# jp-schneider/awesome

Hardware: AMD Instinct MI355X
Metric: INR-fits/sec (256x256 grid, convexity prior) (higher is better)
Workload: dtype f32; 1 GPU; 1 x 256x256 synthetic convex blob per GPU, ConvexNextNet(h=130,L=1), SE(sigmoid) mean, Adam lr 2e-3, clamp, E=2000 full-batch steps (BASELINE configs[1]); images_per_gpu=1, grid=256x256, epochs_per_fit=2000, parallelism=dp1 (independent fits)

## Files before the change

awesome_amd/csrc/flow.h:

```cpp
#pragma once
#include "icnn_step.h"
#include <stdlib.h>

namespace {

constexpr float LEAKY_SLOPE = 0.01f;

struct FlowMap {
    int W, K;
    int nb_stride;
    int p_nb, p_scale, FP;
    int e_cp_stride;
    int e_nb, e_scale, FE;
    float slope;
};

__host__ __device__ inline FlowMap make_flow_map(int W, int K, float slope = LEAKY_SLOPE) {
    FlowMap m;
    m.W = W;
    m.K = K;
    m.slope = slope;
    m.nb_stride = 3 * W + 3;
    m.p_nb = 6;
    m.p_scale = m.p_nb + 2 * K * m.nb_stride;
// ... 514 lines not shown
    float* opt;
    float* grads_out;
    const float* slab1;
    const float* slab2;
    const float* lr_hdr;
    long long hdr_stride;
    InrOptDesc opt_desc;
    FlowMap m;
    int blocks1, S1, chunks, Wp;
    int t;
    double bc1;
    float bc2_sqrt, one_minus_b1, one_minus_b2, wd_g;
    int mode;
    const int32_t* status;
    const float* gscale;
    const float* loss_slabs;
    int loss_wgs;
    long long loss_PS;
};

__device__ __forceinline__ float block_sum256(float v, float* sm, const int tid) {
    v = sum_over_groups(sum_over_points(v));
    __syncthreads();
    if ((tid & 63) == 0) sm[tid >> 6] = v;
    __syncthreads();
    return ((sm[0] + sm[1]) + sm[2]) + sm[3];
}
__device__ __forceinline__ float block_sum256(float v, float* sm) { return block_sum256(v, sm, threadIdx.x); }

constexpr int LOSS_GROUPS = 16;
__device__ __forceinline__ float loss_column_group_sum(const float* __restrict__ sl, const int wgs, const size_t PS, const int grp) {
    float lp = 0.f;
    int w = grp;
    for (; w + 15 * LOSS_GROUPS < wgs; w += 16 * LOSS_GROUPS) {
        float q[16];
#pragma unroll
        for (int k = 0; k < 16; ++k) q[k] = sl[(size_t)(w + k * LOSS_GROUPS) * PS];
#pragma unroll
        for (int k = 0; k < 16; ++k) lp += q[k];
    }
    for (; w < wgs; w += LOSS_GROUPS) lp += sl[(size_t)w * PS];
    return lp;
}

__device__ __forceinline__ bool frozen_in_launch(const float* __restrict__ loss_slabs, const int wgs, const long long PS,
                                                 const float* __restrict__ hdr0, const long long hdr_stride, const int t, const int img,
                                                 const int tid) {
    __shared__ float redl[LOSS_GROUPS];
    if (tid < LOSS_GROUPS) redl[tid] = loss_column_group_sum(loss_slabs + (size_t)img * wgs * PS, wgs, (size_t)PS, tid);
    __syncthreads();
    float loss_now = 0.f;
#pragma unroll
    for (int k = 0; k < LOSS_GROUPS; ++k) loss_now += redl[k];
    const bool bad_before = hdr0 != nullptr && hdr0[(size_t)img * hdr_stride + 6 + (t & 1)] != 0.f;
    return bad_before || !isfinite(loss_now);
}

__device__ __forceinline__ float adam_apply(const FlowUpdArgs& u, float gmul, float p, float g, float lr, float wd, float* m_, float* v_) {
    g = g * gmul;
    if (wd != 0.f) g = __fadd_rn(g, __fmul_rn(wd, p));
    float m = *m_, v = *v_;
    m = __fadd_rn(m, __fmul_rn(u.one_minus_b1, __fsub_rn(g, m)));
    v = __fadd_rn(__fmul_rn(v, u.opt_desc.beta2), __fmul_rn(__fmul_rn(u.one_minus_b2, g), g));
    const float step_size = (float)((double)lr / u.bc1);
    const float denom = __fadd_rn(__fdiv_rn(__fsqrt_rn(v), u.bc2_sqrt), u.opt_desc.eps);
    *m_ = m;
    *v_ = v;
    return __fadd_rn(p, __fdiv_rn(__fmul_rn(-step_size, m), denom));
}

template <int BATCH>
__device__ __forceinline__ void flow_update_body(const FlowUpdArgs& u, const int nb, const int img, const int tid) {
    __shared__ float sm[4];
    const float gmul = u.gscale != nullptr ? u.gscale[img] : 1.f;
    const FlowMap& m = u.m;
    const bool frozen = !isfinite(gmul) ||
                        ((u.mode == 0 && u.loss_slabs != nullptr)
                             ? frozen_in_launch(u.loss_slabs, u.loss_wgs, u.loss_PS, u.lr_hdr, u.hdr_stride, u.t, img, tid)
                             : ((u.lr_hdr != nullptr && u.lr_hdr[(size_t)img * u.hdr_stride + 6 + ((u.t + 1) & 1)] != 0.f) ||
                                (u.status != nullptr && u.status[img] != INR_STATUS_OK)));
    const int mode = (u.mode == 0 && frozen) ? 2 : u.mode;
    const int W = m.W, K = m.K;
    float* __restrict__ fp = u.FP + (size_t)img * m.FP;
    float* __restrict__ fe = u.FE + (size_t)img * m.FE;
    float* __restrict__ om = u.opt ? u.opt + (size_t)img * 2 * m.FP : nullptr;
    float* __restrict__ ov = om ? om + m.FP : nullptr;
    float* __restrict__ go = u.grads_out ? u.grads_out + (size_t)img * m.FP : nullptr;
    const float lr = u.lr_hdr ? u.lr_hdr[(size_t)img * u.hdr_stride + (u.t & 1)] : u.opt_desc.lr;
    if (nb < 2 * K) {
        const int pb = m.p_nb + nb * m.nb_stride;
        const int eb = m.e_nb + (nb >> 1) * m.e_cp_stride + (nb & 1);
        const int i = nb >> 1, net = nb & 1;
        const bool on = tid < W;
// ... 144 lines not shown
```

awesome_amd/csrc/icnn_step.h:

```cpp
#pragma once
#include <hip/hip_runtime.h>
#include <stdint.h>
#include <math.h>

#include <type_traits>

#include "inrfit.h"

typedef float f32x4 __attribute__((ext_vector_type(4)));
typedef float f32x2 __attribute__((ext_vector_type(2)));

#define MFMA16(a, b, c) __builtin_amdgcn_mfma_f32_16x16x4f32((a), (b), (c), 0, 0, 0)
__device__ __forceinline__ float relu0(float x) { return __int_as_float(max(__float_as_int(x), 0)); }
constexpr float INV_2PI = 0.15915494309189535f;
__device__ __forceinline__ float hw_sin(float x) { return __builtin_amdgcn_sinf(__builtin_amdgcn_fractf(x * INV_2PI)); }
__device__ __forceinline__ float hw_cos(float x) { return __builtin_amdgcn_cosf(__builtin_amdgcn_fractf(x * INV_2PI)); }
template <int ACT>
__device__ __forceinline__ float act0_f(float pre, float omega) {
    if constexpr (ACT == INR_ACT_COS) return hw_cos(pre);
    else if constexpr (ACT == INR_ACT_SIN) return hw_sin(omega * pre);
    else return relu0(pre);
}
template <int ACT>
__device__ __forceinline__ float dact0_f(float pre, float omega) {
// ... 164 lines not shown
        }
    }
    if (j < m.p_bo) {
        slot[0] = m.off_wo + (j - m.p_wo);
        return 1;
    }
    slot[0] = m.off_sc + (j - m.p_bo);
    return 1;
}

struct StepArgs {
    const float* wimg;
    const float* targets;
    const float* coef;
    float* slabs;
    float* logits;
    float* dcoords;
    InrGridDesc grid;
    long long N;
    int n_images, wgs, PS, loss_kind;
    float act_omega;
    const float* seg;
    float c_align;
    int data_count;
    int use_noneclass;
    float noneclass;
    int align_soft;
    int align_begin;
};

// ... 722 lines not shown
        }
        for (int i = tid; i < HM * NEXT; i += WG_THREADS) {
            const int row = i / NEXT, e = i - row * NEXT;
            const float v = wsum(SC_L0 + row * 4 + e);
            if (e == 0) slab[G::SL_TILE + G::P_BIN + row] = v;
            else slab[G::SL_TILE + G::P_WIN + row * C + (e - 1)] = v;
        }
        if (tid < HR * NEXT) {
            const int u = tid / NEXT, e = tid - u * NEXT;
            const float v = wsum(SC_L0L + u * 4 + e);
            if (e == 0) slab[G::SL_TILE + G::P_BIN + HM + u] = v;
            else slab[G::SL_TILE + G::P_WIN + (HM + u) * C + (e - 1)] = v;
        }
        if (tid < 2 + C) {
            const float v = wsum(SC_SC + tid);
            if (tid == 0) slab[G::SL_LOSS] = v;
            else if (tid == 1) slab[G::slab_col(G::P_BO)] = v;
            else slab[G::slab_col(G::P_SO) + tid - 2] = v;
        }
    }
#if INR_STAMPS
    if (TRAIN && (tid & 63) == 0 && blockIdx.x < 1024) {
        __builtin_amdgcn_s_waitcnt(0);
        const unsigned long long rt_end = __builtin_amdgcn_s_memrealtime();
        if (tid == 0) {
            g_wgtimes[blockIdx.x][0] = rt_entry;
            g_wgtimes[blockIdx.x][1] = rt_loop;
            g_wgtimes[blockIdx.x][2] = rt_loop_end;
        }
        atomicMax(&g_wgtimes[blockIdx.x][3], rt_end);
    }
    if (TRAIN && blockIdx.x == 0 && tid == 0) {
// ... 13 lines not shown
```

awesome_amd/csrc/icnn_step2.h:

```cpp
#pragma once
#include "icnn_step.h"


namespace {

template <int H, int C>
struct Cfg2 {
    using G1 = Cfg<H, C>;
    static constexpr int TM = G1::TM, HM = G1::HM, HR = G1::HR, NEXT = G1::NEXT, NRL = G1::NRL, KG = G1::KG, PT = G1::PT;
    static constexpr int S = G1::S, SA = G1::SA, SB = G1::SB, RPW = G1::RPW;
    static constexpr int ext_pos(int e) { return G1::ext_pos(e); }
    static constexpr int nr_in(int tk) { return G1::nr_in(tk); }
    static constexpr int OFF_SC = 0;
    static constexpr int OFF_WINE = OFF_SC + 8;
    static constexpr int OFF_WIN = OFF_WINE + 4 * PT;
    static constexpr int OFF_BIN = OFF_WIN + C * 16;
    static constexpr int OFF_FLOOR = OFF_BIN + 16;
    static constexpr int OFF_WO = OFF_FLOOR + 16;
    static constexpr int OFF_WCT0 = OFF_WO + PT;
    static constexpr int OFF_WCT1 = OFF_WCT0 + HR * PT;
    static constexpr int WREG = round_up(H * S + 16, 256);
    static constexpr int OFF_W0 = round_up(OFF_WCT1 + HR * PT, 4);
    static constexpr int OFF_W1 = OFF_W0 + WREG;
    static constexpr int IMG_FLOATS = OFF_W1 + WREG;
// ... 705 lines not shown
        }
        for (int i = tid; i < HM * NEXT; i += WG_THREADS) {
            const int row = i / NEXT, e = i - row * NEXT;
            const float v = wsum(SC_L0 + row * 4 + e);
            if (e == 0) slab[G::SL_IN + G::P_BIN + row] = v;
            else slab[G::SL_IN + G::P_WIN + row * C + (e - 1)] = v;
        }
        if (tid < HR * NEXT) {
            const int u = tid / NEXT, e = tid - u * NEXT;
            const float v = wsum(SC_L0L + u * 4 + e);
            if (e == 0) slab[G::SL_IN + G::P_BIN + HM + u] = v;
            else slab[G::SL_IN + G::P_WIN + (HM + u) * C + (e - 1)] = v;
        }
        if (tid < 2 + C) {
            const float v = wsum(SC_SC + tid);
            if (tid == 0) slab[G::SL_LOSS] = v;
            else if (tid == 1) slab[G::SL_WO + (G::P_BO - G::P_WO)] = v;
            else slab[G::SL_WO + (G::P_SO - G::P_WO) + tid - 2] = v;
        }
    }
}

}
```

awesome_amd/csrc/inrfit.hip:

```cpp
#include "icnn_step.h"
#include "icnn_step2.h"
#include "flow.h"
#include "rnvp.h"
#include "joint_loss.h"
#include "wide.h"
#include "star.h"
#include "cnnseg.h"
#include "fcseg.h"

#include <type_traits>
#include <vector>

namespace {

constexpr int UPD_RANGES = WIDE_MAX_LAYERS + 1;
struct UpdArgs {
    float* wimg;
    ImgMap img;
    float* params;
    float* opt_state;
    const float* slabs;
    float* loss_hist;
    float* grads_out;
    float* loss_out;
    int32_t* status;
    InrOptDesc opt;
    int P, PS, wgs, n_images;
    int Pu, hu;
    int t;
    double bc1;
    float bc2_sqrt;
    float one_minus_b1, one_minus_b2;
    int hist_idx, hist_stride;
    int mode;
    int clamp_lo[UPD_RANGES], clamp_hi[UPD_RANGES];
    int freeze_lo[UPD_RANGES], freeze_hi[UPD_RANGES];
// ... 26 lines not shown
        if (j < m.p_s[k] + H * C) {
            const int q = j - m.p_s[k], o = q / C;
            return o < h ? base_u + h * h + h + q : -1;
        }
    }
    if (j < m.p_bo) {
        const int i = j - m.p_wo;
        return i < h ? base_u + i : -1;
    }
    return base_u + h + (j - m.p_bo);
}

constexpr int UPD_MAX_PARAMS = 256;
constexpr int UPD_GROUPS = 16;

inline int upd_params_per_block(int cols, int reserve = 0) {
    const int cus = 256 - reserve;
    int ppb = ((cols + cus - 1) / cus + 3) / 4 * 4;
    if (ppb < 16) ppb = 16;
    if (ppb > UPD_MAX_PARAMS) ppb = UPD_MAX_PARAMS;
    return ppb;
}
inline dim3 upd_grid(int cols, int n_images, int reserve = 0) {
    const int ppb = upd_params_per_block(cols, reserve);
    return dim3((cols + ppb - 1) / ppb, n_images);
}
inline dim3 upd_block(int cols, int reserve = 0) { return dim3(upd_params_per_block(cols, reserve) / 4, UPD_GROUPS); }

#if INR_STAMPS
__device__ unsigned long long g_updtimes[512][4];
#define UPD_STAMP(k)                                                                                          \
    if (threadIdx.x == 0 && threadIdx.y == 0 && img == 0 && bx < 512) {                                       \
        __builtin_amdgcn_s_waitcnt(0);                                                                        \
        g_updtimes[bx][k] = __builtin_amdgcn_s_memrealtime();                                                 \
    }
#else
#define UPD_STAMP(k)
#endif
static_assert(UPD_GROUPS == LOSS_GROUPS, "the loss column is summed in the update's group order");
__device__ __forceinline__ void icnn_update_body(const UpdArgs& u, const int bx, const int img) {
    const int tx = threadIdx.x, grp = threadIdx.y;
    const int ppb = 4 * blockDim.x;
    __shared__ float red[UPD_GROUPS][UPD_MAX_PARAMS];
    __shared__ float redl[UPD_GROUPS];
    UPD_STAMP(0);
    const int jl = grp * blockDim.x + tx;
    const int j = jl < ppb ? slab_param_of_col(u.img, bx * ppb + jl) : -1;
    const int ju = (j >= 0 && j < u.P) ? user_param_index(u.img, u.hu, j) : -1;
    float* __restrict__ st = u.opt_state + (size_t)img * (2 * (size_t)u.Pu + INR_OPT_HEADER_FLOATS);
    float* __restrict__ hdr = st + 2 * (size_t)u.Pu;
    float p_old = 0.f, m_old = 0.f, v_old = 0.f, lr_now = 0.f;
    bool bad_before = false;
    if (u.mode == 0 && j >= 0) {
        bad_before = hdr[6 + (u.t & 1)] != 0.f;
        lr_now = hdr[u.t & 1];
        if (ju >= 0) {
            p_old = u.params[(size_t)img * u.Pu + ju];
            m_old = st[ju];
            v_old = st[u.Pu + ju];
        }
    }
    {
        const int j4 = bx * ppb + 4 * tx;
        f32x4 part = f32x4{0.f, 0.f, 0.f, 0.f};
        if (j4 < u.PS && slab_param_of_col(u.img, j4) >= 0) {
            const float* __restrict__ sl = u.slabs + (size_t)img * u.wgs * u.PS + j4;
            int w = grp;
            for (; w + 15 * UPD_GROUPS < u.wgs; w += 16 * UPD_GROUPS) {
                f32x4 q[16];
#pragma unroll
                for (int k = 0; k < 16; ++k) q[k] = *(const f32x4*)(sl + (size_t)(w + k * UPD_GROUPS) * u.PS);
#pragma unroll
                for (int k = 0; k < 16; ++k) part += q[k];
            }
            for (; w < u.wgs; w += UPD_GROUPS) part += *(const f32x4*)(sl + (size_t)w * u.PS);
        }
        *(f32x4*)&red[grp][4 * tx] = part;
        if (u.mode == 0 && tx == 0) {
            redl[grp] = loss_column_group_sum(u.slabs + (size_t)img * u.wgs * u.PS + (u.img.sl_cols - 1), u.wgs, (size_t)u.PS, grp);
        }
    }
    UPD_STAMP(1);
    __syncthreads();
    if (j < 0) return;
    float gsum = 0.f;
#pragma unroll
    for (int k = 0; k < UPD_GROUPS; ++k) gsum += red[k][jl];
    if (u.gscale != nullptr && j < u.P) gsum *= u.gscale[img];

    UPD_STAMP(2);
    if (u.mode == 1) {
        if (ju >= 0) u.grads_out[(size_t)img * u.Pu + ju] = gsum;
        else if (j == u.P) u.loss_out[img] = gsum;
        return;
// ... 64 lines not shown
        if (in) p = fmaxf(p, 0.f);
    }
    u.params[(size_t)img * u.Pu + ju] = p;
    if (u.wimg != nullptr) {
        int slot[2];
        const int ns = image_slots(u.img, j, slot);
        float* __restrict__ wi = u.wimg + (size_t)img * u.img.floats;
        wi[slot[0]] = p;
        if (ns > 1) wi[slot[1]] = p;
    }
    st[ju] = m;
    st[u.Pu + ju] = v;
    UPD_STAMP(3);
}

__global__ __launch_bounds__(UPD_MAX_PARAMS / 4 * UPD_GROUPS) void icnn_update_kernel(const UpdArgs u) { icnn_update_body(u, blockIdx.x, blockIdx.y); }

constexpr int UPD_UNION_MAX_THREADS = 768;
__global__ __launch_bounds__(UPD_UNION_MAX_THREADS) void cdn_update_kernel(const UpdArgs ui, const FlowUpdArgs uf, const int nbi) {
    if ((int)blockIdx.x < nbi) {
        icnn_update_body(ui, blockIdx.x, blockIdx.y);
        return;
    }
    const int tid = threadIdx.y * blockDim.x + threadIdx.x;
    if (tid >= 256) return;
    flow_update_body<32>(uf, (int)blockIdx.x - nbi, blockIdx.y, tid);
}
template <int C>
__global__ __launch_bounds__(UPD_UNION_MAX_THREADS) void pcn_update_kernel(const UpdArgs ui, const RnvpUpdArgs ur, const int nbi) {
    if ((int)blockIdx.x < nbi) {
        icnn_update_body(ui, blockIdx.x, blockIdx.y);
        return;
    }
    const int tid = threadIdx.y * blockDim.x + threadIdx.x;
    if (tid >= 256) return;
    rnvp_update_body<C>(ur, (int)blockIdx.x - nbi, blockIdx.y, tid);
}
inline bool upd_union_ok(int cols, int reserve) {
    const dim3 b = upd_block(cols, reserve);
    const int n = (int)(b.x * b.y);
    static const bool off = getenv("INRFIT_SPLIT_UPDATES") != nullptr;
    return !off && n >= 256 && n <= UPD_UNION_MAX_THREADS;
}

__global__ __launch_bounds__(256) void pack_image_kernel(float* __restrict__ wimg, const ImgMap m) {
    float* __restrict__ dst = wimg + (size_t)blockIdx.y * m.floats;
// ... 238 lines not shown
        return INR_ELAUNCH;
    for (int k = 1; k < 3; ++k) {
        if (hipFuncSetAttribute((const void*)e->train_act[k], hipFuncAttributeMaxDynamicSharedMemorySize, e->lds_bytes) != hipSuccess ||
            hipFuncSetAttribute((const void*)e->fwd_act[k], hipFuncAttributeMaxDynamicSharedMemorySize, e->lds_bytes) != hipSuccess)
            return INR_ELAUNCH;
    }
    return INR_OK;
}

constexpr int INR_SLAB_BUFFERS = 4;

struct Workspace {
    float* coef;
    float* wimg;
    float* slabs;
    float* slabs0;
    long long slab_floats;
    int wgs, PS;
    long long bytes;
    void set_step(int it) { slabs = slabs0 + (size_t)(it % INR_SLAB_BUFFERS) * slab_floats; }
    int act0 = INR_ACT_RELU;
    float act_omega = 0.f;
    int hu = 0, Pu = 0;
    void set_user(const KernelEntry* e, const InrModelDesc* m) {
        hu = m ? m->n_hidden : e->h;
        const long long h = hu, c = e->c, l = e->l;
        Pu = (int)(h * c + h + l * (h * h + h + h * c) + h + 1 + c);
    }
};

Workspace carve(const KernelEntry* e, long long n_points, int n_images, void* base) {
    Workspace w;
    w.wgs = wgs_per_image(n_points, n_images);
    w.PS = (e->img.sl_cols + 31) / 32 * 32;
    const long long coef_bytes = ((long long)n_images * 2 * 4 + 255) / 256 * 256;
    const long long img_bytes = ((long long)n_images * e->img.floats * 4 + 255) / 256 * 256;
    w.slab_floats = ((long long)n_images * w.wgs * w.PS + 63) / 64 * 64;
    const long long slab_bytes = w.slab_floats * 4 * INR_SLAB_BUFFERS;
    w.coef = (float*)base;
    w.wimg = (float*)((char*)base + coef_bytes);
    w.slabs0 = w.slabs = (float*)((char*)base + coef_bytes + img_bytes);
    w.bytes = coef_bytes + img_bytes + slab_bytes;
    return w;
}

}

__global__ __launch_bounds__(256) void mfma_stream_kernel(float* __restrict__ sink, int iters) {
    f32x4 acc[8];
#pragma unroll
    for (int t = 0; t < 8; ++t) acc[t] = f32x4{0.f, 0.f, 0.f, 0.f};
    f32x4 av[8], bv;
    unsigned h = (blockIdx.x * 256u + threadIdx.x) * 2654435761u + 12345u;
    auto rnd = [&]() { h = h * 1664525u + 1013904223u; return (float)(int)(h >> 8) * (1.f / 8388608.f) - 1.f; };
#pragma unroll
    for (int t = 0; t < 8; ++t)
// ... 323 lines not shown
                       int loss_kind, int n_images, float* logits, hipStream_t s, float* dcoords = nullptr,
                       const float* align_seg = nullptr, float c_align = 0.f, const StepMask& mask = StepMask{}) {
    StepArgs a{};
    a.dcoords = dcoords;
    a.seg = align_seg;
    a.c_align = c_align;
    a.data_count = (int)(mask.data_count > 0 ? mask.data_count : grid->n_points);
    a.use_noneclass = mask.use_noneclass;
    a.noneclass = mask.noneclass;
    a.align_soft = mask.align_soft;
    a.align_begin = (int)mask.align_begin;
    a.wimg = w.wimg;
    a.targets = targets;
    a.coef = w.coef;
    a.slabs = w.slabs;
    a.logits = logits;
    a.grid = *grid;
    a.N = grid->n_points;
    a.n_images = n_images;
    a.wgs = w.wgs;
    a.PS = w.PS;
    a.loss_kind = loss_kind;
    a.act_omega = w.act_omega;
    if (dcoords && w.act0 != INR_ACT_RELU) return INR_EUNSUPPORTED;
    hipLaunchKernelGGL(train ? (dcoords ? e->train_dx : e->train_act[w.act0]) : e->fwd_act[w.act0], dim3((unsigned)(n_images * w.wgs)),
                       dim3(WG_THREADS), e->lds_bytes, s, a);
    return hipGetLastError() == hipSuccess ? INR_OK : INR_ELAUNCH;
}

struct StepTiming {
// ... 21 lines not shown
static int check_loss(const InrLossDesc* l) {
    if (!l) return INR_EINVAL;
    if (l->kind != INR_LOSS_SE && l->kind != INR_LOSS_BCE && l->kind != INR_LOSS_EXTERNAL) return INR_EINVAL;
    if (l->weight_mode < INR_WEIGHT_NONE || l->weight_mode > INR_WEIGHT_EXPLICIT) return INR_EINVAL;
    return INR_OK;
}

static UpdArgs make_upd_args(const KernelEntry* e, const Workspace& w, float* params, float* opt_state, float* loss_hist,
                             int32_t* status, const InrOptDesc* opt, int n_images, int steps) {
    UpdArgs u{};
    u.wimg = w.wimg;
    u.img = e->img;
    u.params = params;
    u.opt_state = opt_state;
    u.slabs = w.slabs;
    u.loss_hist = loss_hist;
    u.status = status;
    u.opt = *opt;
    u.P = e->P;
    u.Pu = w.Pu;
    u.hu = w.hu;
    u.PS = w.PS;
    u.wgs = w.wgs;
    u.n_images = n_images;
    u.hist_stride = steps;
    u.one_minus_b1 = (float)(1.0 - (double)opt->beta1);
    u.one_minus_b2 = (float)(1.0 - (double)opt->beta2);
    u.mode = 0;
    for (int k = 0; k < UPD_RANGES; ++k) u.clamp_lo[k] = u.clamp_hi[k] = 0;
    for (int k = 0; k < e->img.L; ++k) {
// ... 13 lines not shown
    return u;
}

static void bias_corrections(const InrOptDesc* opt, int t, double* bc1, float* bc2_sqrt) {
    *bc1 = 1.0 - pow((double)opt->beta1, (double)t);
    *bc2_sqrt = (float)sqrt(1.0 - pow((double)opt->beta2, (double)t));
}

static void set_step_consts(UpdArgs& u, const InrOptDesc* opt, int t, int hist_idx = 0) {
    u.t = t;
    bias_corrections(opt, t, &u.bc1, &u.bc2_sqrt);
    u.hist_idx = hist_idx;
}

static void launch_icnn_update(const KernelEntry* e, const UpdArgs& u, hipStream_t s) {
    hipLaunchKernelGGL(icnn_update_kernel, upd_grid(e->img.sl_cols, u.n_images), upd_block(e->img.sl_cols), 0, s, u);
}

static int launch_icnn_update_timed(const KernelEntry* e, const UpdArgs& u, hipStream_t s) {
    if (!g_timing.on || (int)g_timing.evu.size() >= 2 * g_timing.max_samples) {
        launch_icnn_update(e, u, s);
        return INR_OK;
    }
    hipEvent_t a, b;
    if (hipEventCreate(&a) != hipSuccess || hipEventCreate(&b) != hipSuccess) return INR_ELAUNCH;
    (void)hipEventRecord(a, s);
    launch_icnn_update(e, u, s);
    (void)hipEventRecord(b, s);
    g_timing.evu.push_back(a);
    g_timing.evu.push_back(b);
    return INR_OK;
// ... 18 lines not shown
}

static void launch_reduce(const KernelEntry* e, const Workspace& w, int n_images, float* grads, float* loss_out, hipStream_t s) {
    UpdArgs u{};
    u.img = e->img;
    u.slabs = w.slabs;
    u.grads_out = grads;
    u.loss_out = loss_out;
    u.P = e->P;
    u.Pu = w.Pu;
    u.hu = w.hu;
    u.PS = w.PS;
    u.wgs = w.wgs;
    u.n_images = n_images;
    u.mode = 1;
    hipLaunchKernelGGL(icnn_update_kernel, upd_grid(e->img.sl_cols, n_images), upd_block(e->img.sl_cols), 0, s, u);
}


static bool use_wide(const InrModelDesc* m) { return find_entry(m) == nullptr && wide_shape_ok(m); }

static int wide_prepare(const InrModelDesc* model, const InrGridDesc* grid, int n_images, void* workspace, int64_t workspace_bytes,
                        WideMap* m, WideWs* w, float** coef_all, hipStream_t s) {
    if (!workspace || !grid_ok(grid, n_images, 0x7fffffffLL / WIDE_MAX_HIDDEN * 64)) return INR_EINVAL;
    if (model->act0 < INR_ACT_RELU || model->act0 > INR_ACT_SIN) return INR_EINVAL;
    *m = make_wide_map(model);
    const bool pre0 = model->act0 != INR_ACT_RELU;
    if (workspace_bytes < wide_total_bytes(*m, grid->n_points, pre0, n_images)) return INR_EWORKSPACE;
    *w = carve_wide(*m, grid->n_points, pre0, workspace);
    *coef_all = (float*)((char*)workspace + w->bytes);
    (void)s;
// ... 38 lines not shown

static UpdArgs wide_upd_args(const WideMap& m, const float* grads, const InrOptDesc* opt, int steps) {
    UpdArgs u{};
    u.img.identity = 1;
    u.img.H = m.h; u.img.C = m.C; u.img.L = m.L; u.img.P = m.P; u.img.sl_cols = m.P + 1;
    u.opt = *opt;
    u.P = u.Pu = m.P;
    u.hu = m.h;
    u.PS = (m.P + 1 + 31) / 32 * 32;
    u.wgs = 1;
    u.n_images = 1;
    u.hist_stride = steps;
    u.one_minus_b1 = (float)(1.0 - (double)opt->beta1);
    u.one_minus_b2 = (float)(1.0 - (double)opt->beta2);
    u.slabs = grads;
    for (int k = 0; k < UPD_RANGES; ++k) u.clamp_lo[k] = u.clamp_hi[k] = u.freeze_lo[k] = u.freeze_hi[k] = 0;
    for (int k = 0; k < m.L; ++k) {
        u.clamp_lo[k] = m.p_w(k); u.clamp_hi[k] = m.p_w(k) + m.h * m.kin(k);
        u.freeze_lo[k] = m.p_s(k); u.freeze_hi[k] = m.p_s(k) + m.h * m.C;
    }
    u.clamp_lo[UPD_RANGES - 1] = m.p_wo(); u.clamp_hi[UPD_RANGES - 1] = m.p_wo() + m.O * m.hl();
    u.freeze_lo[UPD_RANGES - 1] = m.p_so(); u.freeze_hi[UPD_RANGES - 1] = m.p_so() + m.O * m.C;
    u.input_hi = m.p_w(0);
    return u;
}
static void launch_wide_update(const WideMap& m, const UpdArgs& u, hipStream_t s) {
    hipLaunchKernelGGL(icnn_update_kernel, upd_grid(m.P + 1, 1), upd_block(m.P + 1), 0, s, u);
}

static int wide_fit(const InrModelDesc* model, float* params, float* opt_state, const InrGridDesc* grid, const float* targets,
                    const InrLossDesc* loss, const InrOptDesc* opt, int n_images, int steps, int step0, float* loss_hist,
                    float* final_logits, int32_t* status, void* workspace, int64_t workspace_bytes, hipStream_t s) {
    WideMap m;
    WideWs w;
    float* coef;
    int rc = wide_prepare(model, grid, n_images, workspace, workspace_bytes, &m, &w, &coef, s);
    if (rc) return rc;
    const long long N = grid->n_points, ON = (long long)m.O * N;
    if (m.O > 1 && loss->weight_mode != INR_WEIGHT_NONE && loss->weight_mode != INR_WEIGHT_EXPLICIT) return INR_EINVAL;
    hipLaunchKernelGGL(loss_coef_kernel, dim3(n_images), dim3(256), 0, s, targets, ON, *loss, coef, 1.f);
    hipLaunchKernelGGL(opt_init_kernel, dim3(n_images), dim3(64), 0, s, opt_state, m.P, *opt, step0);
    if (status && hipMemsetAsync(status, 0, sizeof(int32_t) * n_images, s) != hipSuccess) return INR_ELAUNCH;
// ... 186 lines not shown
    return u;
}

static void launch_flow_update_args(const InrFlowDesc* f, int n_images, const FlowUpdArgs& u, hipStream_t s) {
    hipLaunchKernelGGL(flow_update_kernel, dim3(2 * f->num_coupling + 1, n_images), dim3(256), 0, s, u);
}

void launch_flow_update(const CdnWs& w, const InrFlowDesc* f, int n_images, int mode, float* FP, float* grads_out, hipStream_t s) {
    launch_flow_update_args(f, n_images, make_flow_upd_args(w, mode, FP, nullptr, grads_out, nullptr, 0.f, 0, nullptr, 0), s);
}

static void launch_cdn_update(const KernelEntry* e, const UpdArgs& ui, FlowUpdArgs uf, const InrFlowDesc* f, int n_images, hipStream_t s) {
    const int nbf = 2 * f->num_coupling + 1;
    const dim3 gi = upd_grid(e->img.sl_cols, n_images, nbf);
    uf.status = nullptr;
    uf.loss_slabs = ui.slabs + (e->img.sl_cols - 1);
    uf.loss_wgs = ui.wgs;
    uf.loss_PS = ui.PS;
    hipLaunchKernelGGL(cdn_update_kernel, dim3(gi.x + nbf, n_images), upd_block(e->img.sl_cols, nbf), 0, s, ui, uf, (int)gi.x);
}

static void launch_flow_fwd(const CdnWs& w, const InrGridDesc* grid, int n_images, float* out, hipStream_t s) {
    FlowFwdArgs a{};
    a.FE = w.FE;
    a.xd = out;
    a.grid = *grid;
    a.N = grid->n_points;
    a.m = w.fm;
    const dim3 g(w.sf.blocks, n_images), b(w.sf.threads);
    const size_t lds = (w.fm.FE + 64) * sizeof(float);
    if (w.sf.U == 1 && w.sf.Q == 2) hipLaunchKernelGGL((flow_fwd_kernel<2, 1>), g, b, lds, s, a);
    else if (w.sf.U == 4 && w.sf.Q == 2) hipLaunchKernelGGL((flow_fwd_kernel<2, 4>), g, b, lds, s, a);
    else if (w.sf.U == 4 && w.sf.Q == 4) hipLaunchKernelGGL((flow_fwd_kernel<4, 4>), g, b, lds, s, a);
    else if (w.sf.U == 2 && w.sf.Q == 2) hipLaunchKernelGGL((flow_fwd_kernel<2, 2>), g, b, lds, s, a);
// ... 391 lines not shown
    u.t = t;
    if (od && t > 0) {
        bias_corrections(od, t, &u.bc1, &u.bc2_sqrt);
        u.one_minus_b1 = (float)(1.0 - (double)od->beta1);
        u.one_minus_b2 = (float)(1.0 - (double)od->beta2);
    }
    u.wd_flow = wd_flow;
    u.mode = mode;
    return u;
}

static void launch_pcn_update(const KernelEntry* e, const PcnWs& w, const UpdArgs& ui, RnvpUpdArgs ur, int n_images, hipStream_t s) {
    const int nbf = w.rm.F + 1;
    const dim3 gi = upd_grid(e->img.sl_cols, n_images, nbf), g(gi.x + nbf, n_images), b = upd_block(e->img.sl_cols, nbf);
    ur.status = nullptr;
    ur.loss_slabs = ui.slabs + (e->img.sl_cols - 1);
    ur.loss_wgs = ui.wgs;
    ur.loss_PS = ui.PS;
    if (w.rm.C == 2) hipLaunchKernelGGL(pcn_update_kernel<2>, g, b, 0, s, ui, ur, (int)gi.x);
    else hipLaunchKernelGGL(pcn_update_kernel<3>, g, b, 0, s, ui, ur, (int)gi.x);
}

static void launch_rnvp_update_args(const PcnWs& w, int n_images, const RnvpUpdArgs& u, hipStream_t s) {
    const dim3 g(w.rm.F + 1, n_images);
    if (w.rm.C == 2) hipLaunchKernelGGL(rnvp_update_kernel<2>, g, dim3(256), 0, s, u);
    else hipLaunchKernelGGL(rnvp_update_kernel<3>, g, dim3(256), 0, s, u);
}

void launch_rnvp_grads(const PcnWs& w, int n_images, float* rp, float* grads_out, hipStream_t s) {
    launch_rnvp_update_args(w, n_images, make_rnvp_upd_args(w, n_images, 1, rp, nullptr, grads_out, nullptr, 0.f, 0, nullptr, 0, nullptr), s);
}

static bool pcn_wide_shape(const InrModelDesc* m) { return use_wide(m) && m->act0 == INR_ACT_RELU && !wide_desc_general(m); }

struct PcnWideWs {
// ... 543 lines not shown
            const InrLossDesc* loss, const InrOptDesc* opt, int n_images, int steps, int step0, float* loss_hist, float* final_logits,
            int32_t* status, void* workspace, int64_t workspace_bytes, hipStream_t s) {
    const KernelEntry* e;
    int rc = d.check(model, grid, n_images, workspace, workspace_bytes, &e);
    if (rc) return rc;
    hipLaunchKernelGGL(loss_coef_kernel, dim3(n_images), dim3(256), 0, s, targets, (long long)grid->n_points, *loss, d.icnn.coef, 1.f);
    hipLaunchKernelGGL(opt_init_kernel, dim3(n_images), dim3(64), 0, s, opt_state, d.icnn.Pu, *opt, step0);
    if (status && hipMemsetAsync(status, 0, sizeof(int32_t) * n_images, s) != hipSuccess) return INR_ELAUNCH;
    if ((rc = launch_pack(e, d.icnn, params, n_images, s))) return rc;
    d.begin(s);
    UpdArgs u = make_upd_args(e, d.icnn, params, opt_state, loss_hist, status, opt, n_images, steps);
    const bool gate_logits = final_logits && opt->logits_at_last_forward && steps > 0;
    for (int it = 0; it < steps; ++it) {
        d.icnn.set_step(step0 + it);
        u.slabs = d.icnn.slabs;
        set_step_consts(u, opt, step0 + it + 1, it);
        float* logits = gate_logits && it == steps - 1 ? final_logits : nullptr;
        d.forward(true, it > 0, s);
        if constexpr (std::is_same<D, IcnnOnly>::value) {
            if ((rc = launch_step_timed(e, d.icnn, &d.dgrid, targets, loss->kind, n_images, s, logits))) return rc;
            if ((rc = launch_icnn_update_timed(e, u, s))) return rc;
        } else {
            if ((rc = launch_step(e, d.icnn, true, &d.dgrid, targets, loss->kind, n_images, logits, s, d.dxd))) return rc;
            d.update(e, u, true, s);
        }
    }
    if (hipGetLastError() != hipSuccess) return INR_ELAUNCH;
    if (final_logits && !gate_logits) {
        d.forward(false, false, s);
        return launch_step(e, d.icnn, false, &d.dgrid, nullptr, 0, n_images, final_logits, s);
// ... 951 lines not shown
```

awesome_amd/csrc/rnvp.h:

```cpp
#pragma once
#include "flow.h"

#ifndef RNVP_FWD_CLAMP
#define RNVP_FWD_CLAMP 1
#endif

namespace {

constexpr int RNVP_MAX_FLOWS = 32;
constexpr int RNVP_REC = 8;
constexpr int RNVP_TAIL = 16;
constexpr int RNVP_HDR = 16;

struct RnvpMap {
    int C, HID, F;
    int net;
    int pf;
    int RP;
    int fl;
    int LDSF;
    int HIDp;
    int A;
    int out_fn;
    float out_scale;
// ... 835 lines not shown
    int blocks1, S1, chunks;
    int t;
    double bc1;
    float bc2_sqrt, one_minus_b1, one_minus_b2;
    float wd_flow;
    int mode;
    int skip_linear;
    const float* lossp;
    int lossp_blocks;
    float loss_scale;
    float* loss_hist;
    int hist_idx, hist_stride;
    float* RE;
    int unit_linear;
    const float* gscale;
    const float* loss_slabs;
    int loss_wgs;
    long long loss_PS;
};

__device__ __forceinline__ float opt_apply(const RnvpUpdArgs& u, float gmul, float p, float g, float lr, float wd, float* m_, float* v_) {
    g = g * gmul;
    if (wd != 0.f) g = __fadd_rn(g, __fmul_rn(wd, p));
    float m = *m_, v = *v_;
    m = __fadd_rn(m, __fmul_rn(u.one_minus_b1, __fsub_rn(g, m)));
    const float clr = (float)((double)lr / u.bc1);
    if (u.opt_desc.kind == INR_OPT_ADAM) {
        v = __fadd_rn(__fmul_rn(v, u.opt_desc.beta2), __fmul_rn(__fmul_rn(u.one_minus_b2, g), g));
        const float denom = __fadd_rn(__fdiv_rn(__fsqrt_rn(v), u.bc2_sqrt), u.opt_desc.eps);
        p = __fadd_rn(p, __fdiv_rn(__fmul_rn(-clr, m), denom));
    } else {
        v = fmaxf(__fmul_rn(v, u.opt_desc.beta2), __fadd_rn(fabsf(g), u.opt_desc.eps));
        p = __fadd_rn(p, __fdiv_rn(__fmul_rn(-clr, m), v));
    }
    *m_ = m;
    *v_ = v;
    return p;
}

template <int C>
__device__ __forceinline__ void rnvp_update_body(const RnvpUpdArgs& u, const int f, const int img, const int tid) {
    __shared__ float sm[4];
    __shared__ float tot[4 * 3 + 2 * 3];
    const float gmul = u.gscale != nullptr ? u.gscale[img] : 1.f;
    const RnvpMap& m = u.m;
    const int F = m.F, HID = m.HID;
    const bool frozen = !isfinite(gmul) ||
                        (u.loss_slabs != nullptr
                             ? frozen_in_launch(u.loss_slabs, u.loss_wgs, u.loss_PS, u.lr_hdr, u.hdr_stride, u.t, img, tid)
                             : ((u.lr_hdr != nullptr && u.lr_hdr[(size_t)img * u.hdr_stride + 6 + ((u.t + 1) & 1)] != 0.f) ||
                                (u.status != nullptr && u.status[img] != INR_STATUS_OK)));
    float* __restrict__ rp = u.RP + (size_t)img * m.RP;
    float* __restrict__ om = u.opt ? u.opt + (size_t)img * 2 * m.RP : nullptr;
    float* __restrict__ ov = om ? om + m.RP : nullptr;
    float* __restrict__ go = u.grads_out ? u.grads_out + (size_t)img * m.RP : nullptr;
    const float lr = u.lr_hdr ? u.lr_hdr[(size_t)img * u.hdr_stride + (u.t & 1)] : u.opt_desc.lr;
    const int k0 = f < F ? f * 4 * C : F * 4 * C, nk = f < F ? 4 * C : 2 * C;
    {
        __shared__ float wsum[4][4 * 3];
        float part[4 * C];
#pragma unroll
        for (int k = 0; k < 4 * C; ++k) part[k] = 0.f;
        int b = tid;
        for (; b + 768 < u.blocks1; b += 1024) {
// ... 338 lines not shown
```

Measured before the change: 6.528 fits/s.

## Store per-workgroup loss contiguously and rebalance update blocks across CUs by lines

```diff
diff --git a/awesome_amd/csrc/flow.h b/awesome_amd/csrc/flow.h
--- a/awesome_amd/csrc/flow.h
+++ b/awesome_amd/csrc/flow.h
@@ -552,9 +552,9 @@
     int mode;
     const int32_t* status;
     const float* gscale;
-    const float* loss_slabs;
+    const float* loss_part;
     int loss_wgs;
-    long long loss_PS;
+    long long loss_stride;
 };
 
 __device__ __forceinline__ float block_sum256(float v, float* sm, const int tid) {
@@ -567,25 +567,25 @@
 __device__ __forceinline__ float block_sum256(float v, float* sm) { return block_sum256(v, sm, threadIdx.x); }
 
 constexpr int LOSS_GROUPS = 16;
-__device__ __forceinline__ float loss_column_group_sum(const float* __restrict__ sl, const int wgs, const size_t PS, const int grp) {
+__device__ __forceinline__ float loss_column_group_sum(const float* __restrict__ sl, const int wgs, const size_t stride, const int grp) {
     float lp = 0.f;
     int w = grp;
     for (; w + 15 * LOSS_GROUPS < wgs; w += 16 * LOSS_GROUPS) {
         float q[16];
 #pragma unroll
-        for (int k = 0; k < 16; ++k) q[k] = sl[(size_t)(w + k * LOSS_GROUPS) * PS];
+        for (int k = 0; k < 16; ++k) q[k] = sl[(size_t)(w + k * LOSS_GROUPS) * stride];
 #pragma unroll
         for (int k = 0; k < 16; ++k) lp += q[k];
     }
-    for (; w < wgs; w += LOSS_GROUPS) lp += sl[(size_t)w * PS];
+    for (; w < wgs; w += LOSS_GROUPS) lp += sl[(size_t)w * stride];
     return lp;
 }
 
-__device__ __forceinline__ bool frozen_in_launch(const float* __restrict__ loss_slabs, const int wgs, const long long PS,
+__device__ __forceinline__ bool frozen_in_launch(const float* __restrict__ loss_part, const int wgs, const long long stride,
                                                  const float* __restrict__ hdr0, const long long hdr_stride, const int t, const int img,
                                                  const int tid) {
     __shared__ float redl[LOSS_GROUPS];
-    if (tid < LOSS_GROUPS) redl[tid] = loss_column_group_sum(loss_slabs + (size_t)img * wgs * PS, wgs, (size_t)PS, tid);
+    if (tid < LOSS_GROUPS) redl[tid] = loss_column_group_sum(loss_part + (size_t)img * wgs * stride, wgs, (size_t)stride, tid);
     __syncthreads();
     float loss_now = 0.f;
 #pragma unroll
@@ -613,8 +613,8 @@
     const float gmul = u.gscale != nullptr ? u.gscale[img] : 1.f;
     const FlowMap& m = u.m;
     const bool frozen = !isfinite(gmul) ||
-                        ((u.mode == 0 && u.loss_slabs != nullptr)
-                             ? frozen_in_launch(u.loss_slabs, u.loss_wgs, u.loss_PS, u.lr_hdr, u.hdr_stride, u.t, img, tid)
+                        ((u.mode == 0 && u.loss_part != nullptr)
+                             ? frozen_in_launch(u.loss_part, u.loss_wgs, u.loss_stride, u.lr_hdr, u.hdr_stride, u.t, img, tid)
                              : ((u.lr_hdr != nullptr && u.lr_hdr[(size_t)img * u.hdr_stride + 6 + ((u.t + 1) & 1)] != 0.f) ||
                                 (u.status != nullptr && u.status[img] != INR_STATUS_OK)));
     const int mode = (u.mode == 0 && frozen) ? 2 : u.mode;
diff --git a/awesome_amd/csrc/icnn_step.h b/awesome_amd/csrc/icnn_step.h
--- a/awesome_amd/csrc/icnn_step.h
+++ b/awesome_amd/csrc/icnn_step.h
@@ -202,6 +202,7 @@
     const float* targets;
     const float* coef;
     float* slabs;
+    float* loss_part;
     float* logits;
     float* dcoords;
     InrGridDesc grid;
@@ -954,8 +955,10 @@
         }
         if (tid < 2 + C) {
             const float v = wsum(SC_SC + tid);
-            if (tid == 0) slab[G::SL_LOSS] = v;
-            else if (tid == 1) slab[G::slab_col(G::P_BO)] = v;
+            if (tid == 0) {
+                slab[G::SL_LOSS] = v;
+                a.loss_part[(size_t)img * a.wgs + wg] = v;
+            } else if (tid == 1) slab[G::slab_col(G::P_BO)] = v;
             else slab[G::slab_col(G::P_SO) + tid - 2] = v;
         }
     }
diff --git a/awesome_amd/csrc/icnn_step2.h b/awesome_amd/csrc/icnn_step2.h
--- a/awesome_amd/csrc/icnn_step2.h
+++ b/awesome_amd/csrc/icnn_step2.h
@@ -743,8 +743,10 @@
         }
         if (tid < 2 + C) {
             const float v = wsum(SC_SC + tid);
-            if (tid == 0) slab[G::SL_LOSS] = v;
-            else if (tid == 1) slab[G::SL_WO + (G::P_BO - G::P_WO)] = v;
+            if (tid == 0) {
+                slab[G::SL_LOSS] = v;
+                a.loss_part[(size_t)img * a.wgs + wg] = v;
+            } else if (tid == 1) slab[G::SL_WO + (G::P_BO - G::P_WO)] = v;
             else slab[G::SL_WO + (G::P_SO - G::P_WO) + tid - 2] = v;
         }
     }
diff --git a/awesome_amd/csrc/inrfit.hip b/awesome_amd/csrc/inrfit.hip
--- a/awesome_amd/csrc/inrfit.hip
+++ b/awesome_amd/csrc/inrfit.hip
@@ -20,6 +20,8 @@
     float* params;
     float* opt_state;
     const float* slabs;
+    const float* loss_part;
+    long long loss_stride;
     float* loss_hist;
     float* grads_out;
     float* loss_out;
@@ -76,18 +78,32 @@
 constexpr int UPD_MAX_PARAMS = 256;
 constexpr int UPD_GROUPS = 16;
 
-inline int upd_params_per_block(int cols, int reserve = 0) {
-    const int cus = 256 - reserve;
-    int ppb = ((cols + cus - 1) / cus + 3) / 4 * 4;
-    if (ppb < 16) ppb = 16;
-    if (ppb > UPD_MAX_PARAMS) ppb = UPD_MAX_PARAMS;
-    return ppb;
-}
-inline dim3 upd_grid(int cols, int n_images, int reserve = 0) {
-    const int ppb = upd_params_per_block(cols, reserve);
-    return dim3((cols + ppb - 1) / ppb, n_images);
-}
-inline dim3 upd_block(int cols, int reserve = 0) { return dim3(upd_params_per_block(cols, reserve) / 4, UPD_GROUPS); }
+constexpr int UPD_LINE = 32;
+
+struct UpdSplit {
+    int ppb;
+    int n_wide;
+    int blocks;
+};
+inline UpdSplit upd_split(int cols, int reserve = 0) {
+    static const int forced = getenv("INRFIT_UPD_LINES") ? atoi(getenv("INRFIT_UPD_LINES")) : 0;
+    const int cus = 256 - reserve, lines = (cols + UPD_LINE - 1) / UPD_LINE, max_lpb = UPD_MAX_PARAMS / UPD_LINE;
+    int lpb = forced > 0 ? forced : (lines + cus - 1) / cus;
+    if (lpb < 1) lpb = 1;
+    if (lpb > max_lpb) lpb = max_lpb;
+    UpdSplit sp;
+    sp.ppb = lpb * UPD_LINE;
+    if (forced > 0 || lpb == 1 || lines >= lpb * cus) {
+        sp.blocks = (lines + lpb - 1) / lpb;
+        sp.n_wide = sp.blocks;
+    } else {
+        sp.blocks = cus;
+        sp.n_wide = lines - (lpb - 1) * cus;
+    }
+    return sp;
+}
+inline dim3 upd_grid(int cols, int n_images, int reserve = 0) { return dim3(upd_split(cols, reserve).blocks, n_images); }
+inline dim3 upd_block(int cols, int reserve = 0) { return dim3(upd_split(cols, reserve).ppb / 4, UPD_GROUPS); }
 
 #if INR_STAMPS
 __device__ unsigned long long g_updtimes[512][4];
@@ -100,14 +116,16 @@
 #define UPD_STAMP(k)
 #endif
 static_assert(UPD_GROUPS == LOSS_GROUPS, "the loss column is summed in the update's group order");
-__device__ __forceinline__ void icnn_update_body(const UpdArgs& u, const int bx, const int img) {
+__device__ __forceinline__ void icnn_update_body(const UpdArgs& u, const int bx, const int img, const int n_wide) {
     const int tx = threadIdx.x, grp = threadIdx.y;
-    const int ppb = 4 * blockDim.x;
+    const int ppbw = 4 * blockDim.x;
+    const int ppb = bx < n_wide ? ppbw : ppbw - UPD_LINE;
+    const int col0 = bx < n_wide ? bx * ppbw : bx * (ppbw - UPD_LINE) + n_wide * UPD_LINE;
     __shared__ float red[UPD_GROUPS][UPD_MAX_PARAMS];
     __shared__ float redl[UPD_GROUPS];
     UPD_STAMP(0);
     const int jl = grp * blockDim.x + tx;
-    const int j = jl < ppb ? slab_param_of_col(u.img, bx * ppb + jl) : -1;
+    const int j = jl < ppb ? slab_param_of_col(u.img, col0 + jl) : -1;
     const int ju = (j >= 0 && j < u.P) ? user_param_index(u.img, u.hu, j) : -1;
     float* __restrict__ st = u.opt_state + (size_t)img * (2 * (size_t)u.Pu + INR_OPT_HEADER_FLOATS);
     float* __restrict__ hdr = st + 2 * (size_t)u.Pu;
@@ -123,9 +141,9 @@
         }
     }
     {
-        const int j4 = bx * ppb + 4 * tx;
+        const int j4 = col0 + 4 * tx;
         f32x4 part = f32x4{0.f, 0.f, 0.f, 0.f};
-        if (j4 < u.PS && slab_param_of_col(u.img, j4) >= 0) {
+        if (4 * tx < ppb && j4 < u.PS && slab_param_of_col(u.img, j4) >= 0) {
             const float* __restrict__ sl = u.slabs + (size_t)img * u.wgs * u.PS + j4;
             int w = grp;
             for (; w + 15 * UPD_GROUPS < u.wgs; w += 16 * UPD_GROUPS) {
@@ -139,7 +157,7 @@
         }
         *(f32x4*)&red[grp][4 * tx] = part;
         if (u.mode == 0 && tx == 0) {
-            redl[grp] = loss_column_group_sum(u.slabs + (size_t)img * u.wgs * u.PS + (u.img.sl_cols - 1), u.wgs, (size_t)u.PS, grp);
+            redl[grp] = loss_column_group_sum(u.loss_part + (size_t)img * u.wgs * u.loss_stride, u.wgs, (size_t)u.loss_stride, grp);
         }
     }
     UPD_STAMP(1);
@@ -234,12 +252,12 @@
     UPD_STAMP(3);
 }
 
-__global__ __launch_bounds__(UPD_MAX_PARAMS / 4 * UPD_GROUPS) void icnn_update_kernel(const UpdArgs u) { icnn_update_body(u, blockIdx.x, blockIdx.y); }
+__global__ __launch_bounds__(UPD_MAX_PARAMS / 4 * UPD_GROUPS) void icnn_update_kernel(const UpdArgs u, const int n_wide) { icnn_update_body(u, blockIdx.x, blockIdx.y, n_wide); }
 
 constexpr int UPD_UNION_MAX_THREADS = 768;
-__global__ __launch_bounds__(UPD_UNION_MAX_THREADS) void cdn_update_kernel(const UpdArgs ui, const FlowUpdArgs uf, const int nbi) {
+__global__ __launch_bounds__(UPD_UNION_MAX_THREADS) void cdn_update_kernel(const UpdArgs ui, const FlowUpdArgs uf, const int nbi, const int n_wide) {
     if ((int)blockIdx.x < nbi) {
-        icnn_update_body(ui, blockIdx.x, blockIdx.y);
+        icnn_update_body(ui, blockIdx.x, blockIdx.y, n_wide);
         return;
     }
     const int tid = threadIdx.y * blockDim.x + threadIdx.x;
@@ -247,9 +265,9 @@
     flow_update_body<32>(uf, (int)blockIdx.x - nbi, blockIdx.y, tid);
 }
 template <int C>
-__global__ __launch_bounds__(UPD_UNION_MAX_THREADS) void pcn_update_kernel(const UpdArgs ui, const RnvpUpdArgs ur, const int nbi) {
+__global__ __launch_bounds__(UPD_UNION_MAX_THREADS) void pcn_update_kernel(const UpdArgs ui, const RnvpUpdArgs ur, const int nbi, const int n_wide) {
     if ((int)blockIdx.x < nbi) {
-        icnn_update_body(ui, blockIdx.x, blockIdx.y);
+        icnn_update_body(ui, blockIdx.x, blockIdx.y, n_wide);
         return;
     }
     const int tid = threadIdx.y * blockDim.x + threadIdx.x;
@@ -518,11 +536,16 @@
     float* coef;
     float* wimg;
     float* slabs;
+    float* loss_part;
     float* slabs0;
     long long slab_floats;
+    long long loss_off;
     int wgs, PS;
     long long bytes;
-    void set_step(int it) { slabs = slabs0 + (size_t)(it % INR_SLAB_BUFFERS) * slab_floats; }
+    void set_step(int it) {
+        slabs = slabs0 + (size_t)(it % INR_SLAB_BUFFERS) * slab_floats;
+        loss_part = slabs + loss_off;
+    }
     int act0 = INR_ACT_RELU;
     float act_omega = 0.f;
     int hu = 0, Pu = 0;
@@ -539,11 +562,13 @@
     w.PS = (e->img.sl_cols + 31) / 32 * 32;
     const long long coef_bytes = ((long long)n_images * 2 * 4 + 255) / 256 * 256;
     const long long img_bytes = ((long long)n_images * e->img.floats * 4 + 255) / 256 * 256;
-    w.slab_floats = ((long long)n_images * w.wgs * w.PS + 63) / 64 * 64;
+    w.loss_off = ((long long)n_images * w.wgs * w.PS + 63) / 64 * 64;
+    w.slab_floats = w.loss_off + ((long long)n_images * w.wgs + 63) / 64 * 64;
     const long long slab_bytes = w.slab_floats * 4 * INR_SLAB_BUFFERS;
     w.coef = (float*)base;
     w.wimg = (float*)((char*)base + coef_bytes);
     w.slabs0 = w.slabs = (float*)((char*)base + coef_bytes + img_bytes);
+    w.loss_part = w.slabs + w.loss_off;
     w.bytes = coef_bytes + img_bytes + slab_bytes;
     return w;
 }
@@ -897,6 +922,7 @@
     a.targets = targets;
     a.coef = w.coef;
     a.slabs = w.slabs;
+    a.loss_part = w.loss_part;
     a.logits = logits;
     a.grid = *grid;
     a.N = grid->n_points;
@@ -948,6 +974,8 @@
     u.params = params;
     u.opt_state = opt_state;
     u.slabs = w.slabs;
+    u.loss_part = w.loss_part;
+    u.loss_stride = 1;
     u.loss_hist = loss_hist;
     u.status = status;
     u.opt = *opt;
@@ -991,7 +1019,7 @@
 }
 
 static void launch_icnn_update(const KernelEntry* e, const UpdArgs& u, hipStream_t s) {
-    hipLaunchKernelGGL(icnn_update_kernel, upd_grid(e->img.sl_cols, u.n_images), upd_block(e->img.sl_cols), 0, s, u);
+    hipLaunchKernelGGL(icnn_update_kernel, upd_grid(e->img.sl_cols, u.n_images), upd_block(e->img.sl_cols), 0, s, u, upd_split(e->img.sl_cols).n_wide);
 }
 
 static int launch_icnn_update_timed(const KernelEntry* e, const UpdArgs& u, hipStream_t s) {
@@ -1040,7 +1068,7 @@
     u.wgs = w.wgs;
     u.n_images = n_images;
     u.mode = 1;
-    hipLaunchKernelGGL(icnn_update_kernel, upd_grid(e->img.sl_cols, n_images), upd_block(e->img.sl_cols), 0, s, u);
+    hipLaunchKernelGGL(icnn_update_kernel, upd_grid(e->img.sl_cols, n_images), upd_block(e->img.sl_cols), 0, s, u, upd_split(e->img.sl_cols).n_wide);
 }
 
 
@@ -1109,6 +1137,8 @@
     u.one_minus_b1 = (float)(1.0 - (double)opt->beta1);
     u.one_minus_b2 = (float)(1.0 - (double)opt->beta2);
     u.slabs = grads;
+    u.loss_part = grads + m.P;
+    u.loss_stride = u.PS;
     for (int k = 0; k < UPD_RANGES; ++k) u.clamp_lo[k] = u.clamp_hi[k] = u.freeze_lo[k] = u.freeze_hi[k] = 0;
     for (int k = 0; k < m.L; ++k) {
         u.clamp_lo[k] = m.p_w(k); u.clamp_hi[k] = m.p_w(k) + m.h * m.kin(k);
@@ -1120,7 +1150,7 @@
     return u;
 }
 static void launch_wide_update(const WideMap& m, const UpdArgs& u, hipStream_t s) {
-    hipLaunchKernelGGL(icnn_update_kernel, upd_grid(m.P + 1, 1), upd_block(m.P + 1), 0, s, u);
+    hipLaunchKernelGGL(icnn_update_kernel, upd_grid(m.P + 1, 1), upd_block(m.P + 1), 0, s, u, upd_split(m.P + 1).n_wide);
 }
 
 static int wide_fit(const InrModelDesc* model, float* params, float* opt_state, const InrGridDesc* grid, const float* targets,
@@ -1337,10 +1367,11 @@
     const int nbf = 2 * f->num_coupling + 1;
     const dim3 gi = upd_grid(e->img.sl_cols, n_images, nbf);
     uf.status = nullptr;
-    uf.loss_slabs = ui.slabs + (e->img.sl_cols - 1);
+    uf.loss_part = ui.loss_part;
     uf.loss_wgs = ui.wgs;
-    uf.loss_PS = ui.PS;
-    hipLaunchKernelGGL(cdn_update_kernel, dim3(gi.x + nbf, n_images), upd_block(e->img.sl_cols, nbf), 0, s, ui, uf, (int)gi.x);
+    uf.loss_stride = ui.loss_stride;
+    hipLaunchKernelGGL(cdn_update_kernel, dim3(gi.x + nbf, n_images), upd_block(e->img.sl_cols, nbf), 0, s, ui, uf, (int)gi.x,
+                       upd_split(e->img.sl_cols, nbf).n_wide);
 }
 
 static void launch_flow_fwd(const CdnWs& w, const InrGridDesc* grid, int n_images, float* out, hipStream_t s) {
@@ -1762,11 +1793,12 @@
     const int nbf = w.rm.F + 1;
     const dim3 gi = upd_grid(e->img.sl_cols, n_images, nbf), g(gi.x + nbf, n_images), b = upd_block(e->img.sl_cols, nbf);
     ur.status = nullptr;
-    ur.loss_slabs = ui.slabs + (e->img.sl_cols - 1);
+    ur.loss_part = ui.loss_part;
     ur.loss_wgs = ui.wgs;
-    ur.loss_PS = ui.PS;
-    if (w.rm.C == 2) hipLaunchKernelGGL(pcn_update_kernel<2>, g, b, 0, s, ui, ur, (int)gi.x);
-    else hipLaunchKernelGGL(pcn_update_kernel<3>, g, b, 0, s, ui, ur, (int)gi.x);
+    ur.loss_stride = ui.loss_stride;
+    const int n_wide = upd_split(e->img.sl_cols, nbf).n_wide;
+    if (w.rm.C == 2) hipLaunchKernelGGL(pcn_update_kernel<2>, g, b, 0, s, ui, ur, (int)gi.x, n_wide);
+    else hipLaunchKernelGGL(pcn_update_kernel<3>, g, b, 0, s, ui, ur, (int)gi.x, n_wide);
 }
 
 static void launch_rnvp_update_args(const PcnWs& w, int n_images, const RnvpUpdArgs& u, hipStream_t s) {
@@ -2340,6 +2372,7 @@
     for (int it = 0; it < steps; ++it) {
         d.icnn.set_step(step0 + it);
         u.slabs = d.icnn.slabs;
+        u.loss_part = d.icnn.loss_part;
         set_step_consts(u, opt, step0 + it + 1, it);
         float* logits = gate_logits && it == steps - 1 ? final_logits : nullptr;
         d.forward(true, it > 0, s);
diff --git a/awesome_amd/csrc/rnvp.h b/awesome_amd/csrc/rnvp.h
--- a/awesome_amd/csrc/rnvp.h
+++ b/awesome_amd/csrc/rnvp.h
@@ -873,9 +873,9 @@
     float* RE;
     int unit_linear;
     const float* gscale;
-    const float* loss_slabs;
+    const float* loss_part;
     int loss_wgs;
-    long long loss_PS;
+    long long loss_stride;
 };
 
 __device__ __forceinline__ float opt_apply(const RnvpUpdArgs& u, float gmul, float p, float g, float lr, float wd, float* m_, float* v_) {
@@ -905,8 +905,8 @@
     const RnvpMap& m = u.m;
     const int F = m.F, HID = m.HID;
     const bool frozen = !isfinite(gmul) ||
-                        (u.loss_slabs != nullptr
-                             ? frozen_in_launch(u.loss_slabs, u.loss_wgs, u.loss_PS, u.lr_hdr, u.hdr_stride, u.t, img, tid)
+                        (u.loss_part != nullptr
+                             ? frozen_in_launch(u.loss_part, u.loss_wgs, u.loss_stride, u.lr_hdr, u.hdr_stride, u.t, img, tid)
                              : ((u.lr_hdr != nullptr && u.lr_hdr[(size_t)img * u.hdr_stride + 6 + ((u.t + 1) & 1)] != 0.f) ||
                                 (u.status != nullptr && u.status[img] != INR_STATUS_OK)));
     float* __restrict__ rp = u.RP + (size_t)img * m.RP;
```

Measured after the change: 6.601 fits/s (median of 6 runs). +1.1%, better.
